# rvignav/diffusion-tts

Measured on AMD Instinct MI355X. Metric: candidate U-Net steps/sec, EDM ImageNet-64 eps-greedy N=64, higher is better.
Workload: dtype f16x3; 1 GPU; EDM ImageNet-64 (ADM 295.9M) eps-greedy search iteration, imagenet scorer, sigma step 5/18; candidates_total=64, candidates_per_gpu=64, scorer=imagenet, scorer_dtype=f16x3, denoiser_dtype=f16x3, graph_replay=True, parity_grade=True, parallelism=candidates sharded x1, 1 all-gather of rewards per step

## Files before the change

### diffusion_tts_amd/build.py

```python
import os
import re
import subprocess
import sys
from concurrent.futures import ThreadPoolExecutor

HERE = os.path.dirname(os.path.abspath(__file__))
CSRC = os.path.join(HERE, 'csrc')
LIB = os.path.join(HERE, 'libdts_hip.so')
SOURCES = ['conv_igemm.hip', 'conv_small.hip', 'groupnorm.hip', 'attention.hip', 'elementwise.hip', 'resample.hip', 'transformer.hip', 'group_rows.hip', 'vit.hip', 'jpeg.hip']
HIPCC = os.environ.get('HIPCC', '/opt/rocm/bin/hipcc')
FLAGS = ['--offload-arch=gfx950', '-O3', '-std=c++17', '-fPIC', '-Wall', '-Wno-unused-function']
EXTRA = {'attention.hip': ['-mllvm', '-amdgpu-mfma-vgpr-form=1']}


def _newer(a, b):
    return (not os.path.exists(b)) or os.path.getmtime(a) > os.path.getmtime(b)


def build(force=False, verbose=False):
    hdrs = [os.path.join(CSRC, 'dts_common.h'), os.path.join(HERE, '..', 'include', 'dts.h')]
    objs, jobs = [], []
    for src in SOURCES:
        s = os.path.join(CSRC, src)
        o = os.path.join(CSRC, src.replace('.hip', '.o'))
        objs.append(o)
        if force or _newer(s, o) or any(_newer(h, o) for h in hdrs):
            jobs.append([HIPCC, *FLAGS, *EXTRA.get(src, []), '-c', s, '-o', o])

    def run(cmd):
        if verbose:
            print(' '.join(cmd), flush=True)
        r = subprocess.run(cmd, capture_output=True, text=True)
        if r.returncode != 0:
            raise RuntimeError(f'hipcc failed: {" ".join(cmd)}\n{r.stdout}\n{r.stderr}')
        return r.stderr

    if jobs and os.path.exists(LIB):
        os.remove(LIB)
    with ThreadPoolExecutor(max_workers=4) as ex:
        for warn in ex.map(run, jobs):
            if verbose and warn.strip():
                print(warn)
    if jobs or force or not os.path.exists(LIB):
        for o in M0_OBJECTS:
            check_m0(os.path.join(CSRC, o))
        run([HIPCC, '--offload-arch=gfx950', '-shared', '-fPIC', '-o', LIB, *objs])
    return LIB


OBJDUMP = os.environ.get('LLVM_OBJDUMP', '/opt/rocm/lib/llvm/bin/llvm-objdump')
READELF = os.environ.get('LLVM_READELF', os.path.join(os.path.dirname(OBJDUMP), 'llvm-readelf'))
M0_OBJECTS = ['conv_igemm.o', 'attention.o']


def _device_object(obj, tmp):
    import glob
    local = os.path.join(tmp, os.path.basename(obj))
    with open(obj, 'rb') as f, open(local, 'wb') as g:
        g.write(f.read())
    subprocess.run([OBJDUMP, '--offloading', local], capture_output=True, text=True, cwd=tmp)
    dev = glob.glob(local + '.*gfx950*')
    if not dev:
        raise RuntimeError('no gfx950 code object found in ' + obj)
    return dev[0]


def check_m0(obj):
    import tempfile
    if not os.path.exists(OBJDUMP):
        print(f'WARNING: {OBJDUMP} not found: the M0 safety check of {os.path.basename(obj)} was SKIPPED (set LLVM_OBJDUMP)', file=sys.stderr)
        return -1
    with tempfile.TemporaryDirectory() as tmp:
        dev = _device_object(obj, tmp)
        dis = subprocess.run([OBJDUMP, '-d', dev], capture_output=True, text=True).stdout
        notes = subprocess.run([READELF, '--notes', dev], capture_output=True, text=True).stdout if os.path.exists(READELF) else ''
    name = os.path.basename(obj)
    ours = re.compile(r'^s_mov_b32 m0, (s\d+|vcc_lo|vcc_hi)$')
    uses, bad, dma_kernels, cur = 0, [], set(), None
    for ln in dis.splitlines():
        m = re.match(r'^[0-9a-f]+ <([^>]+)>:', ln)
        if m:
            cur = m.group(1)
            continue
        code = ln.split('//')[0].strip()
        if 'm0' in code:
            uses += 1
            dma_kernels.add(cur)
            if not ours.match(code):
                bad.append(code)
    if bad or not uses:
        raise RuntimeError(f'{name} code object: {len(bad)} instruction(s) other than our `s_mov_b32 m0, sN` use M0 '
                           f'(first: {bad[:3]}); the M0-clobber shortcut of the LDS-DMA helpers is no longer safe')
    if notes:
        spilled = []
        for blk in re.split(r'\n\s+- \.agpr_count', notes)[1:]:
            g = lambda k: re.search(r'\.%s:\s+(\S+)' % k, blk).group(1)
            if g('name') in dma_kernels and (int(g('private_segment_fixed_size')) != 0 or int(g('vgpr_spill_count')) != 0):
                spilled.append((g('name'), int(g('private_segment_fixed_size')), int(g('vgpr_spill_count'))))
        if spilled:
            raise RuntimeError(f'{name}: LDS-DMA kernels with scratch / VGPR spills (their hand-counted vmcnt waits would no longer hold): {spilled[:3]}')
    else:
        print(f'WARNING: {READELF} not found: the no-scratch check of the LDS-DMA kernels in {name} was SKIPPED', file=sys.stderr)
    return uses


if __name__ == '__main__':
    print(build(force='--force' in sys.argv, verbose=True))
```

### diffusion_tts_amd/csrc/attention.hip

```cpp
#include "dts_common.h"
#include <mutex>
#include <unordered_map>

namespace {

template <typename T> struct AttMma;
template <> struct AttMma<bf16_t> {
  static __device__ __forceinline__ f32x4_t run(const uint4& a, const uint4& b, f32x4_t c) {
    return __builtin_amdgcn_mfma_f32_16x16x32_bf16(__builtin_bit_cast(bf16x8_t, a), __builtin_bit_cast(bf16x8_t, b), c, 0, 0, 0);
  }
  static __device__ __forceinline__ uint32_t pack2(float lo, float hi) { return pack2_bf16(lo, hi); }
  static constexpr uint32_t ONES2 = 0x3F803F80u;
};
template <> struct AttMma<f16_t> {
  static __device__ __forceinline__ f32x4_t run(const uint4& a, const uint4& b, f32x4_t c) {
    return __builtin_amdgcn_mfma_f32_16x16x32_f16(__builtin_bit_cast(f16x8_t, a), __builtin_bit_cast(f16x8_t, b), c, 0, 0, 0);
  }
  static __device__ __forceinline__ uint32_t pack2(float lo, float hi) { return pack2_f16(lo, hi); }
  static constexpr uint32_t ONES2 = 0x3C003C00u;
};

__device__ __forceinline__ float vmax3(float a, float b, float c) {
  float r;
  asm("v_max3_f32 %0, %1, %2, %3" : "=v"(r) : "v"(a), "v"(b), "v"(c));
  return r;
}
__device__ __forceinline__ float vmax2(float a, float b) {
  float r;
  asm("v_max_f32 %0, %1, %2" : "=v"(r) : "v"(a), "v"(b));
  return r;
}

__device__ uint4 g_att_zero[64];

__device__ __forceinline__ void att_glds16(const char* g, uint32_t lds_off) {
  asm volatile("s_mov_b32 m0, %1\n\ts_nop 0\n\tglobal_load_lds_dwordx4 %0, off" : : "v"(g), "s"(lds_off) : "memory", "m0");
}

struct AttP {
  const char* qkv; char* out;
  int n, t, heads, d;
  float scale_log2e;
  int qblocks;
  int xcd_remap;
  int out_split3;
};

__device__ __forceinline__ void att_block(const AttP& p, int& nh, int& qb) {
  int bid = blockIdx.x;
  if (p.xcd_remap) {
    const int nblk = gridDim.x, q = nblk >> 3, r = nblk & 7, xcd = bid & 7, j = bid >> 3;
    bid = (xcd < r ? xcd * (q + 1) : r * (q + 1) + (xcd - r) * q) + j;
  }
  nh = bid / p.qblocks;
  qb = bid - nh * p.qblocks;
}

template <typename T, int D, int QT, int DV = D, bool PREF = true, bool DB = false, bool DMA = false>
__global__ __launch_bounds__(256) void attention16_kernel(const AttP p) {
  static_assert(!DB || PREF, "double buffering rides on the register prefetch");
  static_assert(!DMA || (D == 512 && DV == 256 && QT == 1 && !PREF && !DB), "LDS-DMA staging: the head-dim-512 form only");
  constexpr int ES = 2, ROWB = D * ES + 32;
  constexpr int VROWB = DV * ES + 32;
  constexpr int CH = D / 8;
  constexpr int CHV = DV / 8;
  constexpr int KSTEPS = D / 32;
  constexpr int DT = DV / 16;
  constexpr int NSL = D / DV;
  constexpr bool WIDE = DMA;
  extern __shared__ __attribute__((aligned(16))) char smem[];
  constexpr int BUFB = 64 * ROWB + 64 * VROWB;
  char* sK = smem;
  char* sV = smem + 64 * ROWB;
  const int tid = threadIdx.x, lane = tid & 63, wid = tid >> 6;
  const int lq = lane & 15, lg = lane >> 4;
  int nh, qblk;
  att_block(p, nh, qblk);
  int vs = 0;
  if constexpr (NSL > 1) { vs = nh % NSL; nh /= NSL; }
  const int n = nh / p.heads, head = nh - n * p.heads;
  const int C = p.heads * D;
  const size_t rowstride = (size_t)3 * C * ES;
  const char* base = p.qkv + (size_t)n * p.t * rowstride + (size_t)head * D * ES;
  const int q0 = qblk * (64 * QT) + wid * (16 * QT);

  uint4 qf[QT][KSTEPS];
#pragma unroll
  for (int qt = 0; qt < QT; ++qt)
#pragma unroll
    for (int s = 0; s < KSTEPS; ++s) {
      const int qrow = q0 + qt * 16 + lq;
      qf[qt][s] = make_uint4(0, 0, 0, 0);
      if (qrow < p.t) qf[qt][s] = *reinterpret_cast<const uint4*>(base + (size_t)qrow * rowstride + (lg + 4 * s) * 16);
    }
  const float sc2 = p.scale_log2e;
  f32x4_t o[QT][DT];
  f32x4_t ol[QT];
  const uint4 ones = make_uint4(AttMma<T>::ONES2, AttMma<T>::ONES2, AttMma<T>::ONES2, AttMma<T>::ONES2);
  float m_run[QT];
#pragma unroll
  for (int qt = 0; qt < QT; ++qt) {
    m_run[qt] = -INFINITY; ol[qt] = f32x4_t{0.f, 0.f, 0.f, 0.f};
#pragma unroll
    for (int i = 0; i < DT; ++i) o[qt][i] = f32x4_t{0.f, 0.f, 0.f, 0.f};
  }

  const int ntiles = (p.t + 63) / 64;
  constexpr int NCH = (64 * CH) / 256;
  constexpr int NCHV = (64 * CHV) / 256;
  constexpr int NPF = PREF ? NCH : 1, NPFV = PREF ? NCHV : 1;
  uint4 pk[NPF], pv[NPFV];
  const char* const vbase = base + (size_t)2 * C * ES + (size_t)vs * DV * ES;
#define ATT_LOAD_TILE(key0_)                                                                     \
  _Pragma("unroll") for (int u = 0; u < NCH; ++u) {                                               \
    const int idx = tid + 256 * u, r = idx / CH, c = idx - r * CH;                                \
    pk[u] = make_uint4(0, 0, 0, 0);                                                               \
    if ((key0_) + r < p.t) pk[u] = *reinterpret_cast<const uint4*>(base + (size_t)((key0_) + r) * rowstride + c * 16 + (size_t)C * ES); \
  }                                                                                               \
  _Pragma("unroll") for (int u = 0; u < NCHV; ++u) {                                              \
    const int idx = tid + 256 * u, r = idx / CHV, c = idx - r * CHV;                              \
    pv[u] = make_uint4(0, 0, 0, 0);                                                               \
    if ((key0_) + r < p.t) pv[u] = *reinterpret_cast<const uint4*>(vbase + (size_t)((key0_) + r) * rowstride + c * 16); \
  }
#define ATT_STAGE_TILE(boff_)                                                                     \
  _Pragma("unroll") for (int u = 0; u < NCH; ++u) {                                               \
    const int idx = tid + 256 * u, r = idx / CH, c = idx - r * CH;                                \
    *reinterpret_cast<uint4*>(sK + (boff_) + r * ROWB + c * 16) = pk[u];                          \
  }                                                                                               \
  _Pragma("unroll") for (int u = 0; u < NCHV; ++u) {                                              \
    const int idx = tid + 256 * u, r = idx / CHV, c = idx - r * CHV;                              \
    *reinterpret_cast<uint4*>(sV + (boff_) + r * VROWB + c * 16) = pv[u];                         \
  }
  const uint32_t lds_k = (uint32_t)(uintptr_t)(__attribute__((address_space(3))) char*)sK;
  const uint32_t lds_v = (uint32_t)(uintptr_t)(__attribute__((address_space(3))) char*)sV;
  const char* const zsrc = reinterpret_cast<const char*>(g_att_zero) + lane * 16;
#define ATT_DMA_K(key0_)                                                                         \
  _Pragma("unroll") for (int i = 0; i < 16; ++i) {                                                \
    const int r = wid * 16 + i;                                                                   \
    const char* src = ((key0_) + r < p.t) ? base + (size_t)((key0_) + r) * rowstride + (size_t)C * ES + lane * 16 : zsrc; \
    att_glds16(src, __builtin_amdgcn_readfirstlane(lds_k + r * ROWB));                            \
  }
#define ATT_DMA_V(key0_)                                                                         \
  if (lane < 32) {                                                                                \
    _Pragma("unroll") for (int i = 0; i < 16; ++i) {                                              \
      const int r = wid * 16 + i;                                                                 \
      const char* src = ((key0_) + r < p.t) ? vbase + (size_t)((key0_) + r) * rowstride + lane * 16 : zsrc; \
      att_glds16(src, __builtin_amdgcn_readfirstlane(lds_v + r * VROWB));                         \
    }                                                                                             \
  }
  if constexpr (DMA) { ATT_DMA_K(0); ATT_DMA_V(0); }
  if constexpr (PREF) { ATT_LOAD_TILE(0); }
  if constexpr (DB) {
    ATT_STAGE_TILE(0);
    if (ntiles > 1) { ATT_LOAD_TILE(64); }
  }
  for (int kt = 0; kt < ntiles; ++kt) {
    const int key0 = kt * 64;
    const int boff = DB ? (kt & 1) * BUFB : 0;
    if constexpr (DMA) asm volatile("s_waitcnt vmcnt(16)" ::: "memory");
    __syncthreads();
    if constexpr (DMA) {
    } else if constexpr (DB) {
      if (kt + 1 < ntiles) {
        ATT_STAGE_TILE(BUFB - boff);
        if (kt + 2 < ntiles) { ATT_LOAD_TILE(key0 + 128); }
      }
    } else if constexpr (PREF) {
      ATT_STAGE_TILE(0);
    } else {
#pragma unroll
      for (int u0 = 0; u0 < NCH; u0 += 4) {
        uint4 tk[4];
#pragma unroll
        for (int u = 0; u < 4; ++u) {
          const int idx = tid + 256 * (u0 + u), r = idx / CH, c = idx - r * CH;
          tk[u] = make_uint4(0, 0, 0, 0);
          if (key0 + r < p.t) tk[u] = *reinterpret_cast<const uint4*>(base + (size_t)(key0 + r) * rowstride + c * 16 + (size_t)C * ES);
        }
#pragma unroll
        for (int u = 0; u < 4; ++u) {
          const int idx = tid + 256 * (u0 + u), r = idx / CH, c = idx - r * CH;
          *reinterpret_cast<uint4*>(sK + r * ROWB + c * 16) = tk[u];
        }
      }
#pragma unroll
      for (int u0 = 0; u0 < NCHV; u0 += 4) {
        uint4 tv[4];
#pragma unroll
        for (int u = 0; u < 4; ++u) {
// ... 3 lines not shown
        }
#pragma unroll
        for (int u = 0; u < 4; ++u) {
          const int idx = tid + 256 * (u0 + u), r = idx / CHV, c = idx - r * CHV;
          *reinterpret_cast<uint4*>(sV + r * VROWB + c * 16) = tv[u];
        }
      }
    }
    if constexpr (!DB && !DMA) {
      __syncthreads();
      if constexpr (PREF) { if (kt + 1 < ntiles) { ATT_LOAD_TILE(key0 + 64); } }
    }

    f32x4_t sacc[QT][4];
    if constexpr (WIDE) {
#pragma unroll
      for (int j = 0; j < 4; ++j)
#pragma unroll
        for (int qt = 0; qt < QT; ++qt) sacc[qt][j] = f32x4_t{0.f, 0.f, 0.f, 0.f};
#pragma unroll
      for (int s = 0; s < KSTEPS; ++s) {
        uint4 ka[4];
#pragma unroll
        for (int j = 0; j < 4; ++j) ka[j] = *reinterpret_cast<const uint4*>(sK + boff + (j * 16 + lq) * ROWB + (lg + 4 * s) * 16);
#pragma unroll
        for (int j = 0; j < 4; ++j)
#pragma unroll
          for (int qt = 0; qt < QT; ++qt) sacc[qt][j] = AttMma<T>::run(ka[j], qf[qt][s], sacc[qt][j]);
      }
    } else {
#pragma unroll
    for (int j = 0; j < 4; ++j) {
#pragma unroll
      for (int qt = 0; qt < QT; ++qt) sacc[qt][j] = f32x4_t{0.f, 0.f, 0.f, 0.f};
#pragma unroll
      for (int s = 0; s < KSTEPS; ++s) {
        const uint4 ka = *reinterpret_cast<const uint4*>(sK + boff + (j * 16 + lq) * ROWB + (lg + 4 * s) * 16);
#pragma unroll
        for (int qt = 0; qt < QT; ++qt) sacc[qt][j] = AttMma<T>::run(ka, qf[qt][s], sacc[qt][j]);
      }
    }
    }
    if constexpr (DMA) {
      __syncthreads();
      if (kt + 1 < ntiles) { ATT_DMA_K(key0 + 64); }
    }
    uint4 pb[QT][2];
#pragma unroll
    for (int qt = 0; qt < QT; ++qt) {
      if (key0 + 64 > p.t) {
#pragma unroll
        for (int j = 0; j < 4; ++j)
#pragma unroll
          for (int r = 0; r < 4; ++r)
            if (key0 + j * 16 + lg * 4 + r >= p.t) sacc[qt][j][r] = -INFINITY;
      }
      float tmax = vmax3(sacc[qt][0][0], sacc[qt][0][1], sacc[qt][0][2]);
      tmax = vmax3(tmax, sacc[qt][0][3], sacc[qt][1][0]);
      tmax = vmax3(tmax, sacc[qt][1][1], sacc[qt][1][2]);
      tmax = vmax3(tmax, sacc[qt][1][3], sacc[qt][2][0]);
      tmax = vmax3(tmax, sacc[qt][2][1], sacc[qt][2][2]);
      tmax = vmax3(tmax, sacc[qt][2][3], sacc[qt][3][0]);
      tmax = vmax3(tmax, sacc[qt][3][1], sacc[qt][3][2]);
      tmax = vmax2(tmax, sacc[qt][3][3]);
      {
        const float t16 = __shfl_xor(tmax, 16, 64), t32 = __shfl_xor(tmax, 32, 64), t48 = __shfl_xor(tmax, 48, 64);
        tmax = vmax2(vmax3(tmax, t16, t32), t48);
      }
      const float m_new = vmax2(m_run[qt], tmax);
      const float alpha = __builtin_amdgcn_exp2f((m_run[qt] - m_new) * sc2);
      const float mb = m_new * sc2;
#pragma unroll
      for (int j = 0; j < 4; ++j)
#pragma unroll
        for (int r = 0; r < 4; ++r) sacc[qt][j][r] = __builtin_amdgcn_exp2f(fmaf(sacc[qt][j][r], sc2, -mb));
      m_run[qt] = m_new;
      if (!__all(alpha == 1.0f)) {
#pragma unroll
        for (int i = 0; i < DT; ++i) o[qt][i] *= alpha;
        ol[qt][0] *= alpha;
      }
#pragma unroll
      for (int kk = 0; kk < 2; ++kk) {
        pb[qt][kk].x = AttMma<T>::pack2(sacc[qt][2 * kk][0], sacc[qt][2 * kk][1]);
        pb[qt][kk].y = AttMma<T>::pack2(sacc[qt][2 * kk][2], sacc[qt][2 * kk][3]);
        pb[qt][kk].z = AttMma<T>::pack2(sacc[qt][2 * kk + 1][0], sacc[qt][2 * kk + 1][1]);
        pb[qt][kk].w = AttMma<T>::pack2(sacc[qt][2 * kk + 1][2], sacc[qt][2 * kk + 1][3]);
      }
    }

    if constexpr (DMA) {
      if (kt + 1 < ntiles) asm volatile("s_waitcnt vmcnt(16)" ::: "memory");
      else asm volatile("s_waitcnt vmcnt(0)" ::: "memory");
      __syncthreads();
    }
#pragma unroll
    for (int kk = 0; kk < 2; ++kk) {
      const int rq = (lane & 15) >> 2, rp = lane & 3;
      const char* va = sV + boff + (32 * kk + 4 * lg + rq) * VROWB + rp * 8;
#pragma unroll
      for (int qt = 0; qt < QT; ++qt) ol[qt] = AttMma<T>::run(ones, pb[qt][kk], ol[qt]);
      const char* vb = va + 16 * VROWB;
      if constexpr (WIDE) {
#pragma unroll
        for (int dt0 = 0; dt0 < DT; dt0 += 4) {
          uint4 av[4];
#pragma unroll
          for (int u = 0; u < 4; ++u) {
            const s16x4_t lo = __builtin_amdgcn_ds_read_tr16_b64_v4i16((__attribute__((address_space(3))) s16x4_t*)(va + (dt0 + u) * 32));
            const s16x4_t hi = __builtin_amdgcn_ds_read_tr16_b64_v4i16((__attribute__((address_space(3))) s16x4_t*)(vb + (dt0 + u) * 32));
            const uint2 lo2 = __builtin_bit_cast(uint2, lo), hi2 = __builtin_bit_cast(uint2, hi);
            av[u] = make_uint4(lo2.x, lo2.y, hi2.x, hi2.y);
          }
#pragma unroll
          for (int u = 0; u < 4; ++u)
#pragma unroll
            for (int qt = 0; qt < QT; ++qt) o[qt][dt0 + u] = AttMma<T>::run(av[u], pb[qt][kk], o[qt][dt0 + u]);
        }
      } else {
#pragma unroll
      for (int dt = 0; dt < DT; ++dt) {
        const s16x4_t lo = __builtin_amdgcn_ds_read_tr16_b64_v4i16((__attribute__((address_space(3))) s16x4_t*)(va + dt * 32));
        const s16x4_t hi = __builtin_amdgcn_ds_read_tr16_b64_v4i16((__attribute__((address_space(3))) s16x4_t*)(vb + dt * 32));
        const uint2 lo2 = __builtin_bit_cast(uint2, lo), hi2 = __builtin_bit_cast(uint2, hi);
        const uint4 av = make_uint4(lo2.x, lo2.y, hi2.x, hi2.y);
#pragma unroll
        for (int qt = 0; qt < QT; ++qt) o[qt][dt] = AttMma<T>::run(av, pb[qt][kk], o[qt][dt]);
      }
      }
    }
    if constexpr (DMA) {
      __syncthreads();
      if (kt + 1 < ntiles) { ATT_DMA_V(key0 + 64); }
    }
  }
#pragma unroll
  for (int qt = 0; qt < QT; ++qt) {
    const int qrow = q0 + qt * 16 + lq;
    if (qrow < p.t) {
      const float inv = 1.f / ol[qt][0];
      T* orow = reinterpret_cast<T*>(p.out) + ((size_t)n * p.t + qrow) * C + head * D + vs * DV;
#pragma unroll
      for (int dt = 0; dt < DT; ++dt)
#pragma unroll
        for (int r = 0; r < 4; ++r) st1<T>(orow + dt * 16 + lg * 4 + r, o[qt][dt][r] * inv);
    }
  }
}
#undef ATT_LOAD_TILE
#undef ATT_STAGE_TILE
#undef ATT_DMA_K
#undef ATT_DMA_V

template <int QT, int VAR = 7>
__global__ __launch_bounds__(256) void attention_x3_kernel(const AttP p) {
  using T = f16_t;
  constexpr bool KPRE = (VAR & 1) != 0, SM2 = (VAR & 2) != 0;
  constexpr int D = 64, ES = 2, ROWB = 2 * D * ES + 32, CH = 2 * D / 8, KSTEPS = D / 32, DT = D / 16, NCH = (64 * CH) / 256;
  extern __shared__ __attribute__((aligned(16))) char smem[];
  char* sK = smem;
  char* sV = smem + 64 * ROWB;
  const int tid = threadIdx.x, lane = tid & 63, wid = tid >> 6;
  const int lq = lane & 15, lg = lane >> 4;
  int nh, qblk;
  att_block(p, nh, qblk);
  const int n = nh / p.heads, head = nh - n * p.heads;
  const int C = p.heads * D;
  const size_t rowstride = (size_t)6 * C * ES;
  const size_t LO = (size_t)3 * C * ES;
  const char* base = p.qkv + (size_t)n * p.t * rowstride + (size_t)head * D * ES;
  const int q0 = qblk * (64 * QT) + wid * (16 * QT);
  uint4 qh[QT][KSTEPS], ql[QT][KSTEPS];
#pragma unroll
  for (int qt = 0; qt < QT; ++qt)
#pragma unroll
    for (int s = 0; s < KSTEPS; ++s) {
      const int qrow = q0 + qt * 16 + lq;
      qh[qt][s] = ql[qt][s] = make_uint4(0, 0, 0, 0);
      if (qrow < p.t) {
        qh[qt][s] = *reinterpret_cast<const uint4*>(base + (size_t)qrow * rowstride + (lg + 4 * s) * 16);
        ql[qt][s] = *reinterpret_cast<const uint4*>(base + (size_t)qrow * rowstride + LO + (lg + 4 * s) * 16);
      }
    }
  const float sc2 = p.scale_log2e * (1.0f / 4096.0f);
  f32x4_t o[QT][DT], ol[QT];
  const uint4 ones = make_uint4(AttMma<T>::ONES2, AttMma<T>::ONES2, AttMma<T>::ONES2, AttMma<T>::ONES2);
  float m_run[QT];
#pragma unroll
  for (int qt = 0; qt < QT; ++qt) {
    m_run[qt] = -INFINITY; ol[qt] = f32x4_t{0.f, 0.f, 0.f, 0.f};
#pragma unroll
    for (int i = 0; i < DT; ++i) o[qt][i] = f32x4_t{0.f, 0.f, 0.f, 0.f};
  }
  const int ntiles = (p.t + 63) / 64;
  uint4 pk[NCH], pv[NCH];
  static_assert(CH == 16 && NCH == 4, "tile staging layout");
  typedef unsigned int att_u32x4 __attribute__((ext_vector_type(4)));
  const __amdgpu_buffer_rsrc_t rs_kv = __builtin_amdgcn_make_buffer_rsrc((void*)const_cast<char*>(base), 0, 0x7fff0000, 0x00020000);
  uint32_t koff[NCH];
  {
    const int r = tid >> 4, c = tid & 15;
#pragma unroll
    for (int u = 0; u < NCH; ++u)
      koff[u] = (uint32_t)((size_t)(r + 16 * u) * rowstride + (c < 8 ? 0 : LO) + (size_t)(c & 7) * 16 + (size_t)C * ES);
  }
  const uint32_t v_plane = (uint32_t)((size_t)C * ES);
#define X3_LD(voff_, soff_) __builtin_bit_cast(uint4, (att_u32x4)__builtin_amdgcn_raw_buffer_load_b128(rs_kv, (int)(voff_), (int)(soff_), 0))
#define X3_LOAD_TILE(key0_)                                                                      \
  {                                                                                               \
    const uint32_t so_ = (uint32_t)((size_t)(key0_) * rowstride);                                 \
    if ((key0_) + 64 <= p.t) {                                                                    \
      _Pragma("unroll") for (int u = 0; u < NCH; ++u) { pk[u] = X3_LD(koff[u], so_); pv[u] = X3_LD(koff[u], so_ + v_plane); }      \
    } else {                                                                                      \
      _Pragma("unroll") for (int u = 0; u < NCH; ++u) {                                           \
        const uint32_t vo_ = ((key0_) + (tid >> 4) + 16 * u < p.t) ? koff[u] : 0x80000000u;       \
        pk[u] = X3_LD(vo_, so_); pv[u] = X3_LD(vo_, so_ + v_plane);                               \
      }                                                                                           \
    }                                                                                             \
  }
  const uint32_t st_off = (uint32_t)((tid >> 4) * ROWB + (tid & 15) * 16);
#define X3_STAGE_TILE()                                                                           \
  _Pragma("unroll") for (int u = 0; u < NCH; ++u) {                                               \
    *reinterpret_cast<uint4*>(sK + st_off + u * (16 * ROWB)) = pk[u];                             \
    *reinterpret_cast<uint4*>(sV + st_off + u * (16 * ROWB)) = pv[u];                             \
  }
  X3_LOAD_TILE(0);
  for (int kt = 0; kt < ntiles; ++kt) {
    const int key0 = kt * 64;
    __syncthreads();
    X3_STAGE_TILE();
    __syncthreads();
    if (kt + 1 < ntiles) { X3_LOAD_TILE(key0 + 64); }
    f32x4_t sacc[QT][4];
    uint4 kf[2][KSTEPS][2];
#pragma unroll
    for (int s = 0; s < KSTEPS; ++s) {
      kf[0][s][0] = *reinterpret_cast<const uint4*>(sK + lq * ROWB + (lg + 4 * s) * 16);
      kf[0][s][1] = *reinterpret_cast<const uint4*>(sK + lq * ROWB + D * ES + (lg + 4 * s) * 16);
    }
#pragma unroll
    for (int j = 0; j < 4; ++j) {
#pragma unroll
      for (int qt = 0; qt < QT; ++qt) sacc[qt][j] = f32x4_t{0.f, 0.f, 0.f, 0.f};
      if (KPRE && j < 3) {
#pragma unroll
        for (int s = 0; s < KSTEPS; ++s) {
          kf[(j + 1) & 1][s][0] = *reinterpret_cast<const uint4*>(sK + ((j + 1) * 16 + lq) * ROWB + (lg + 4 * s) * 16);
          kf[(j + 1) & 1][s][1] = *reinterpret_cast<const uint4*>(sK + ((j + 1) * 16 + lq) * ROWB + D * ES + (lg + 4 * s) * 16);
        }
      }
      if constexpr (KPRE) __builtin_amdgcn_sched_barrier(0);
#pragma unroll
      for (int s = 0; s < KSTEPS; ++s) {
        uint4 kh = kf[j & 1][s][0], kl = kf[j & 1][s][1];
        if (!KPRE && j > 0) {
          kh = *reinterpret_cast<const uint4*>(sK + (j * 16 + lq) * ROWB + (lg + 4 * s) * 16);
          kl = *reinterpret_cast<const uint4*>(sK + (j * 16 + lq) * ROWB + D * ES + (lg + 4 * s) * 16);
        }
#pragma unroll
        for (int qt = 0; qt < QT; ++qt) {
          sacc[qt][j] = AttMma<T>::run(kh, qh[qt][s], sacc[qt][j]);
          sacc[qt][j] = AttMma<T>::run(kh, ql[qt][s], sacc[qt][j]);
          sacc[qt][j] = AttMma<T>::run(kl, qh[qt][s], sacc[qt][j]);
        }
      }
    }
#define X3_VFRAG(kk_, dt_, avh_, avl_)                                                                                                    \
  {                                                                                                                                       \
    const char* va_ = sV + (32 * (kk_) + 4 * lg + ((lane & 15) >> 2)) * ROWB + (lane & 3) * 8 + (dt_) * 32;                                \
    const uint2 h0_ = __builtin_bit_cast(uint2, __builtin_amdgcn_ds_read_tr16_b64_v4i16((__attribute__((address_space(3))) s16x4_t*)(va_)));               \
    const uint2 h1_ = __builtin_bit_cast(uint2, __builtin_amdgcn_ds_read_tr16_b64_v4i16((__attribute__((address_space(3))) s16x4_t*)(va_ + 16 * ROWB)));   \
    const uint2 l0_ = __builtin_bit_cast(uint2, __builtin_amdgcn_ds_read_tr16_b64_v4i16((__attribute__((address_space(3))) s16x4_t*)(va_ + D * ES)));      \
    const uint2 l1_ = __builtin_bit_cast(uint2, __builtin_amdgcn_ds_read_tr16_b64_v4i16((__attribute__((address_space(3))) s16x4_t*)(va_ + 16 * ROWB + D * ES))); \
    avh_ = make_uint4(h0_.x, h0_.y, h1_.x, h1_.y); avl_ = make_uint4(l0_.x, l0_.y, l1_.x, l1_.y);                                          \
  }
    constexpr int VPRE = (VAR & 4) ? 2 : 0;
    uint4 vpre[VPRE > 0 ? VPRE : 1][2];
#pragma unroll
    for (int dt = 0; dt < VPRE; ++dt) X3_VFRAG(0, dt, vpre[dt][0], vpre[dt][1]);
    uint4 pbh[QT][2], pbl[QT][2];
    float tmx[QT], t16[QT], t32[QT], t48[QT];
#pragma unroll
    for (int qt = 0; qt < QT; ++qt) {
      if (key0 + 64 > p.t) {
#pragma unroll
        for (int j = 0; j < 4; ++j)
#pragma unroll
          for (int r = 0; r < 4; ++r)
            if (key0 + j * 16 + lg * 4 + r >= p.t) sacc[qt][j][r] = -INFINITY;
      }
      float tmax = vmax3(sacc[qt][0][0], sacc[qt][0][1], sacc[qt][0][2]);
      tmax = vmax3(tmax, sacc[qt][0][3], sacc[qt][1][0]);
      tmax = vmax3(tmax, sacc[qt][1][1], sacc[qt][1][2]);
      tmax = vmax3(tmax, sacc[qt][1][3], sacc[qt][2][0]);
      tmax = vmax3(tmax, sacc[qt][2][1], sacc[qt][2][2]);
      tmax = vmax3(tmax, sacc[qt][2][3], sacc[qt][3][0]);
      tmax = vmax3(tmax, sacc[qt][3][1], sacc[qt][3][2]);
      tmx[qt] = vmax2(tmax, sacc[qt][3][3]);
    }
    if constexpr (SM2) {
#pragma unroll
      for (int qt = 0; qt < QT; ++qt) {
        t16[qt] = __shfl_xor(tmx[qt], 16, 64); t32[qt] = __shfl_xor(tmx[qt], 32, 64); t48[qt] = __shfl_xor(tmx[qt], 48, 64);
      }
    }
#pragma unroll
    for (int qt = 0; qt < QT; ++qt) {
      float tmax;
      if constexpr (SM2) tmax = vmax2(vmax3(tmx[qt], t16[qt], t32[qt]), t48[qt]);
      else { tmax = vmax2(tmx[qt], __shfl_xor(tmx[qt], 16, 64)); tmax = vmax2(tmax, __shfl_xor(tmax, 32, 64)); }
      const float m_new = vmax2(m_run[qt], tmax);
      const float alpha = __builtin_amdgcn_exp2f((m_run[qt] - m_new) * sc2);
      const float mb = m_new * sc2 - 14.0f;
      m_run[qt] = m_new;
      if (!__all(alpha == 1.0f)) {
#pragma unroll
        for (int i = 0; i < DT; ++i) o[qt][i] *= alpha;
        ol[qt][0] *= alpha;
      }
      uint32_t hw_[4][2], lw_[4][2];
#pragma unroll
      for (int j = 0; j < 4; ++j)
#pragma unroll
        for (int r = 0; r < 4; r += 2) {
          const float e0 = __builtin_amdgcn_exp2f(fmaf(sacc[qt][j][r], sc2, -mb));
          const float e1 = __builtin_amdgcn_exp2f(fmaf(sacc[qt][j][r + 1], sc2, -mb));
          const dts_f32x2_t ev = {e0, e1};
          const dts_f16x2_t hv = __builtin_convertvector(ev, dts_f16x2_t);
          const float l0 = __builtin_fmaf((float)hv[0], -1.0f, e0), l1 = __builtin_fmaf((float)hv[1], -1.0f, e1);
          hw_[j][r >> 1] = __builtin_bit_cast(uint32_t, hv);
          lw_[j][r >> 1] = pack2_f16(l0, l1);
        }
#pragma unroll
      for (int kk = 0; kk < 2; ++kk) {
        pbh[qt][kk] = make_uint4(hw_[2 * kk][0], hw_[2 * kk][1], hw_[2 * kk + 1][0], hw_[2 * kk + 1][1]);
        pbl[qt][kk] = make_uint4(lw_[2 * kk][0], lw_[2 * kk][1], lw_[2 * kk + 1][0], lw_[2 * kk + 1][1]);
      }
    }
#pragma unroll
    for (int kk = 0; kk < 2; ++kk) {
#pragma unroll
      for (int qt = 0; qt < QT; ++qt) {
        ol[qt] = AttMma<T>::run(ones, pbh[qt][kk], ol[qt]);
        ol[qt] = AttMma<T>::run(ones, pbl[qt][kk], ol[qt]);
      }
#pragma unroll
      for (int dt = 0; dt < DT; ++dt) {
        uint4 avh, avl;
        if (kk == 0 && dt < VPRE) { avh = vpre[dt][0]; avl = vpre[dt][1]; }
        else X3_VFRAG(kk, dt, avh, avl);
#pragma unroll
        for (int qt = 0; qt < QT; ++qt) {
          o[qt][dt] = AttMma<T>::run(avh, pbh[qt][kk], o[qt][dt]);
          o[qt][dt] = AttMma<T>::run(avh, pbl[qt][kk], o[qt][dt]);
          o[qt][dt] = AttMma<T>::run(avl, pbh[qt][kk], o[qt][dt]);
        }
      }
    }
  }
#undef X3_VFRAG
#undef X3_LOAD_TILE
#undef X3_LD
#undef X3_STAGE_TILE
#pragma unroll
  for (int qt = 0; qt < QT; ++qt) {
    const int qrow = q0 + qt * 16 + lq;
    if (qrow < p.t) {
      const float inv = (1.0f / 64.0f) / ol[qt][0];
      if (p.out_split3) {
        f16_t* orow3 = reinterpret_cast<f16_t*>(p.out) + ((size_t)n * p.t + qrow) * 2 * C;
#pragma unroll
        for (int dt = 0; dt < DT; ++dt) {
          float hi[4], lo[4];
#pragma unroll
          for (int r = 0; r < 4; ++r) {
            float x = o[qt][dt][r] * inv;
            asm volatile("" : "+v"(x));
            x3_split(x, hi[r], lo[r]);
          }
          f16_t* d_ = orow3 + x3_off(head * D + dt * 16 + lg * 4);
          *reinterpret_cast<uint2*>(d_) = make_uint2(pack2_f16(hi[0], hi[1]), pack2_f16(hi[2], hi[3]));
          *reinterpret_cast<uint2*>(d_ + 32) = make_uint2(pack2_f16(lo[0], lo[1]), pack2_f16(lo[2], lo[3]));
        }
      } else {
        float* orow = reinterpret_cast<float*>(p.out) + ((size_t)n * p.t + qrow) * C + head * D;
#pragma unroll
        for (int dt = 0; dt < DT; ++dt)
          *reinterpret_cast<float4*>(orow + dt * 16 + lg * 4) = make_float4(o[qt][dt][0] * inv, o[qt][dt][1] * inv, o[qt][dt][2] * inv, o[qt][dt][3] * inv);
      }
    }
  }
}


template <int D>
__global__ __launch_bounds__(256) void attention32_kernel(const AttP p) {
  constexpr int ES = 4, ROWB = D * ES + 32;
  constexpr int CH = D / 4;
  constexpr int KCH = D / 16;
  constexpr int DT = D / 16;
  extern __shared__ __attribute__((aligned(16))) char smem[];
  char* sK = smem;
  char* sV = smem + 64 * ROWB;
  const int tid = threadIdx.x, lane = tid & 63, wid = tid >> 6;
  const int lq = lane & 15, lg = lane >> 4;
  int nh, qblk;
  att_block(p, nh, qblk);
  const int n = nh / p.heads, head = nh - n * p.heads;
  const int C = p.heads * D;
  const size_t rowstride = (size_t)3 * C * ES;
  const char* base = p.qkv + (size_t)n * p.t * rowstride + (size_t)head * D * ES;
  const int q0 = qblk * 64 + wid * 16;
  const int qrow = q0 + lq;

  f32x4_t o[DT];
#pragma unroll
  for (int i = 0; i < DT; ++i) o[i] = f32x4_t{0.f, 0.f, 0.f, 0.f};
  float m_run = -INFINITY, l_run = 0.f;
  const int ntiles = (p.t + 63) / 64;
  for (int kt = 0; kt < ntiles; ++kt) {
    const int key0 = kt * 64;
    __syncthreads();
    for (int idx = tid; idx < 64 * CH; idx += 256) {
      const int r = idx / CH, c = idx - r * CH;
      uint4 kv = make_uint4(0, 0, 0, 0), vv = make_uint4(0, 0, 0, 0);
      if (key0 + r < p.t) {
        const char* g = base + (size_t)(key0 + r) * rowstride + c * 16;
        kv = *reinterpret_cast<const uint4*>(g + (size_t)C * ES);
        vv = *reinterpret_cast<const uint4*>(g + (size_t)2 * C * ES);
      }
      *reinterpret_cast<uint4*>(sK + r * ROWB + c * 16) = kv;
      *reinterpret_cast<uint4*>(sV + r * ROWB + c * 16) = vv;
    }
    __syncthreads();
    f32x4_t sacc[4];
#pragma unroll
    for (int j = 0; j < 4; ++j) sacc[j] = f32x4_t{0.f, 0.f, 0.f, 0.f};
#pragma unroll
    for (int s = 0; s < KCH; ++s) {
      float4 qv = make_float4(0.f, 0.f, 0.f, 0.f);
      if (qrow < p.t) qv = *reinterpret_cast<const float4*>(base + (size_t)qrow * rowstride + (lg + 4 * s) * 16);
#pragma unroll
      for (int j = 0; j < 4; ++j) {
        const float4 ka = *reinterpret_cast<const float4*>(sK + (j * 16 + lq) * ROWB + (lg + 4 * s) * 16);
        sacc[j] = __builtin_amdgcn_mfma_f32_16x16x4f32(ka.x, qv.x, sacc[j], 0, 0, 0);
        sacc[j] = __builtin_amdgcn_mfma_f32_16x16x4f32(ka.y, qv.y, sacc[j], 0, 0, 0);
        sacc[j] = __builtin_amdgcn_mfma_f32_16x16x4f32(ka.z, qv.z, sacc[j], 0, 0, 0);
        sacc[j] = __builtin_amdgcn_mfma_f32_16x16x4f32(ka.w, qv.w, sacc[j], 0, 0, 0);
      }
    }
    float tmax = -INFINITY;
#pragma unroll
    for (int j = 0; j < 4; ++j)
#pragma unroll
      for (int r = 0; r < 4; ++r) {
        float v = sacc[j][r] * p.scale_log2e;
        if (key0 + j * 16 + lg * 4 + r >= p.t) v = -INFINITY;
        sacc[j][r] = v;
        tmax = fmaxf(tmax, v);
      }
    tmax = fmaxf(tmax, __shfl_xor(tmax, 16, 64));
    tmax = fmaxf(tmax, __shfl_xor(tmax, 32, 64));
    const float m_new = fmaxf(m_run, tmax);
    const float alpha = exp2f(m_run - m_new);
    float psum = 0.f;
#pragma unroll
    for (int j = 0; j < 4; ++j)
#pragma unroll
      for (int r = 0; r < 4; ++r) {
        const float e = exp2f(sacc[j][r] - m_new);
        sacc[j][r] = e;
        psum += e;
      }
    psum += __shfl_xor(psum, 16, 64);
    psum += __shfl_xor(psum, 32, 64);
    l_run = l_run * alpha + psum;
    m_run = m_new;
#pragma unroll
    for (int i = 0; i < DT; ++i) o[i] *= alpha;
#pragma unroll
    for (int j = 0; j < 4; ++j)
#pragma unroll
      for (int r = 0; r < 4; ++r) {
        const char* vrow = sV + (j * 16 + 4 * lg + r) * ROWB + lq * 4;
#pragma unroll
        for (int dt = 0; dt < DT; ++dt) {
          const float va = *reinterpret_cast<const float*>(vrow + dt * 64);
          o[dt] = __builtin_amdgcn_mfma_f32_16x16x4f32(va, sacc[j][r], o[dt], 0, 0, 0);
        }
      }
  }
  if (qrow < p.t) {
    const float inv = 1.f / l_run;
    float* orow = reinterpret_cast<float*>(p.out) + ((size_t)n * p.t + qrow) * C + head * D;
#pragma unroll
    for (int dt = 0; dt < DT; ++dt) {
      const float4 v = make_float4(o[dt][0] * inv, o[dt][1] * inv, o[dt][2] * inv, o[dt][3] * inv);
      *reinterpret_cast<float4*>(orow + dt * 16 + lg * 4) = v;
    }
  }
}

struct AttMaskP {
  const char* qkv; char* out;
  const int32_t* key_len;
  int n, t, heads;
  float scale_log2e;
  int qblocks, xcd_remap, causal;
};

template <typename T>
__global__ __launch_bounds__(256) void attention_masked_kernel(const AttMaskP p) {
  constexpr int D = 64, ES = 2, ROWB = D * ES + 32, CH = D / 8, KSTEPS = D / 32, DT = D / 16, NCH = (64 * CH) / 256;
// ... 58 lines not shown
    if (kt + 1 < ntiles) { ATTM_LOAD_TILE(key0 + 64); }

    f32x4_t sacc[4];
#pragma unroll
    for (int j = 0; j < 4; ++j) {
      sacc[j] = f32x4_t{0.f, 0.f, 0.f, 0.f};
#pragma unroll
      for (int s = 0; s < KSTEPS; ++s) {
        const uint4 ka = *reinterpret_cast<const uint4*>(sK + (j * 16 + lq) * ROWB + (lg + 4 * s) * 16);
        sacc[j] = AttMma<T>::run(ka, qf[s], sacc[j]);
      }
    }
    if (key0 + 64 > kend || (p.causal && key0 + 63 > q0)) {
#pragma unroll
      for (int j = 0; j < 4; ++j)
#pragma unroll
        for (int r = 0; r < 4; ++r)
          if (key0 + j * 16 + lg * 4 + r >= lim) sacc[j][r] = -INFINITY;
    }
    float tmax = vmax3(sacc[0][0], sacc[0][1], sacc[0][2]);
    tmax = vmax3(tmax, sacc[0][3], sacc[1][0]);
    tmax = vmax3(tmax, sacc[1][1], sacc[1][2]);
    tmax = vmax3(tmax, sacc[1][3], sacc[2][0]);
    tmax = vmax3(tmax, sacc[2][1], sacc[2][2]);
    tmax = vmax3(tmax, sacc[2][3], sacc[3][0]);
    tmax = vmax3(tmax, sacc[3][1], sacc[3][2]);
    tmax = vmax2(tmax, sacc[3][3]);
    {
      const float t16 = __shfl_xor(tmax, 16, 64), t32 = __shfl_xor(tmax, 32, 64), t48 = __shfl_xor(tmax, 48, 64);
      tmax = vmax2(vmax3(tmax, t16, t32), t48);
    }
    const float m_new = vmax2(m_run, tmax);
    const float alpha = __builtin_amdgcn_exp2f((m_run - m_new) * sc2);
    const float mb = m_new * sc2;
#pragma unroll
    for (int j = 0; j < 4; ++j)
#pragma unroll
      for (int r = 0; r < 4; ++r) sacc[j][r] = __builtin_amdgcn_exp2f(fmaf(sacc[j][r], sc2, -mb));
    m_run = m_new;
    if (!__all(alpha == 1.0f)) {
#pragma unroll
      for (int i = 0; i < DT; ++i) o[i] *= alpha;
      ol[0] *= alpha;
    }
    uint4 pb[2];
#pragma unroll
    for (int kk = 0; kk < 2; ++kk) {
      pb[kk].x = AttMma<T>::pack2(sacc[2 * kk][0], sacc[2 * kk][1]);
      pb[kk].y = AttMma<T>::pack2(sacc[2 * kk][2], sacc[2 * kk][3]);
      pb[kk].z = AttMma<T>::pack2(sacc[2 * kk + 1][0], sacc[2 * kk + 1][1]);
      pb[kk].w = AttMma<T>::pack2(sacc[2 * kk + 1][2], sacc[2 * kk + 1][3]);
    }
#pragma unroll
    for (int kk = 0; kk < 2; ++kk) {
      const int rq = (lane & 15) >> 2, rp = lane & 3;
      const char* va = sV + (32 * kk + 4 * lg + rq) * ROWB + rp * 8;
      const char* vb = va + 16 * ROWB;
      ol = AttMma<T>::run(ones, pb[kk], ol);
#pragma unroll
      for (int dt = 0; dt < DT; ++dt) {
        const s16x4_t lo = __builtin_amdgcn_ds_read_tr16_b64_v4i16((__attribute__((address_space(3))) s16x4_t*)(va + dt * 32));
        const s16x4_t hi = __builtin_amdgcn_ds_read_tr16_b64_v4i16((__attribute__((address_space(3))) s16x4_t*)(vb + dt * 32));
        const uint2 lo2 = __builtin_bit_cast(uint2, lo), hi2 = __builtin_bit_cast(uint2, hi);
        o[dt] = AttMma<T>::run(make_uint4(lo2.x, lo2.y, hi2.x, hi2.y), pb[kk], o[dt]);
      }
    }
  }
#undef ATTM_LOAD_TILE
  if (qrow < p.t) {
    const float inv = 1.f / ol[0];
    T* orow = reinterpret_cast<T*>(p.out) + ((size_t)n * p.t + qrow) * C + head * D;
#pragma unroll
    for (int dt = 0; dt < DT; ++dt)
#pragma unroll
      for (int r = 0; r < 4; ++r) st1<T>(orow + dt * 16 + lg * 4 + r, o[dt][r] * inv);
  }
}

template <typename T>
int att_masked(AttMaskP p, hipStream_t st) {
  p.qblocks = (p.t + 63) / 64;
  p.xcd_remap = dts_knob_get(DTS_KNOB_ATT_XCD) != 0;
  const long long nblk = (long long)p.qblocks * p.n * p.heads;
  DTS_CHECK_ARG(nblk < (1ll << 31), "dts_attention_masked: grid too large");
  hipLaunchKernelGGL(attention_masked_kernel<T>, dim3((unsigned)nblk), dim3(256), 0, st, p);
  DTS_CHECK_LAUNCH("dts_attention_masked");
  return DTS_OK;
}

template <typename K>
int launch_att(K kernel, const AttP& p0, size_t lds, hipStream_t st, int qblock = 64, int slices = 1) {
  {
    static std::mutex mu;
    static std::unordered_map<uintptr_t, size_t> done;
    int dev = 0;
    if (hipGetDevice(&dev) != hipSuccess) dev = 0;
    std::lock_guard<std::mutex> lk(mu);
    size_t& have = done[reinterpret_cast<uintptr_t>(reinterpret_cast<const void*>(kernel)) ^ ((uintptr_t)(dev + 1) << 56)];
    if (lds > have) {
      (void)hipFuncSetAttribute(reinterpret_cast<const void*>(kernel), hipFuncAttributeMaxDynamicSharedMemorySize, (int)lds);
      have = lds;
    }
  }
  AttP p = p0;
  p.qblocks = (p.t + qblock - 1) / qblock;
  p.xcd_remap = dts_knob_get(DTS_KNOB_ATT_XCD) != 0;
  const long long nblk = (long long)p.qblocks * p.n * p.heads * slices;
  DTS_CHECK_ARG(nblk < (1ll << 31), "dts_attention: grid too large");
  hipLaunchKernelGGL(kernel, dim3((unsigned)nblk), dim3(256), lds, st, p);
  DTS_CHECK_LAUNCH("dts_attention");
  return DTS_OK;
}

template <typename T>
int att16(const AttP& p, hipStream_t st) {
  const int g_att_qt = dts_knob_get(DTS_KNOB_ATT_QT) > 0 ? dts_knob_get(DTS_KNOB_ATT_QT) : 0;
  const size_t lds = (size_t)2 * 64 * (p.d * 2 + 32);
  const bool db = dts_knob_get(DTS_KNOB_ATT_DB) == 1 && p.t > 64;
  switch (p.d) {
    case 64:
      if (g_att_qt == 2 || (g_att_qt == 0 && p.t >= 256 && (long long)((p.t + 127) / 128) * p.n * p.heads >= 512))
        return db ? launch_att(attention16_kernel<T, 64, 2, 64, true, true>, p, 2 * lds, st, 128)
                  : launch_att(attention16_kernel<T, 64, 2>, p, lds, st, 128);
      return db ? launch_att(attention16_kernel<T, 64, 1, 64, true, true>, p, 2 * lds, st) : launch_att(attention16_kernel<T, 64, 1>, p, lds, st);
    case 128:
      return db ? launch_att(attention16_kernel<T, 128, 1, 128, true, true>, p, 2 * lds, st) : launch_att(attention16_kernel<T, 128, 1>, p, lds, st);
    case 256: return launch_att(attention16_kernel<T, 256, 1>, p, lds, st);
    case 512:
      if (dts_knob_get(DTS_KNOB_ATT_DB) == 2)
        return launch_att(attention16_kernel<T, 512, 1, 256, false>, p, (size_t)64 * (512 * 2 + 32) + (size_t)64 * (256 * 2 + 32), st, 64, 2);
      return launch_att(attention16_kernel<T, 512, 1, 256, false, false, true>, p, (size_t)64 * (512 * 2 + 32) + (size_t)64 * (256 * 2 + 32), st, 64, 2);
  }
  return DTS_ERR_UNSUPPORTED;
}

int att32(const AttP& p, hipStream_t st) {
  const size_t lds = (size_t)2 * 64 * (p.d * 4 + 32);
  switch (p.d) {
    case 64: return launch_att(attention32_kernel<64>, p, lds, st);
    case 128: return launch_att(attention32_kernel<128>, p, lds, st);
    case 256: return launch_att(attention32_kernel<256>, p, lds, st);
  }
  return DTS_ERR_UNSUPPORTED;
}

}

extern "C" int dts_attention_x3(const void* qkv_split, void* out, int out_split3, int n, int t, int heads, int d, float scale, dts_stream s) {
  DTS_CHECK_ARG(qkv_split && out, "dts_attention_x3: null pointer");
  DTS_CHECK_ARG(n > 0 && t > 0 && heads > 0, "dts_attention_x3: bad shape");
  DTS_CHECK_ARG(d == 64, "dts_attention_x3: head dim %d unsupported (64; other sizes take dts_attention in DTS_F32)", d);
  DTS_CHECK_ARG((long long)t * 6 * heads * d * 2 < (1ll << 31), "dts_attention_x3: %d tokens x %d heads exceed the 2 GiB a sample's rows may span", t, heads);
  AttP p{(const char*)qkv_split, (char*)out, n, t, heads, d, scale * 1.4426950408889634f, 0, 1, out_split3 ? 1 : 0};
  const size_t lds = (size_t)2 * 64 * (2 * 64 * 2 + 32);
  const int qt = dts_knob_get(DTS_KNOB_ATT_QT);
  const bool two = qt == 2 || (qt != 1 && t >= 512 && (long long)((t + 127) / 128) * n * heads >= 512);
  const int var = (dts_knob_get(DTS_KNOB_ATT_DB) >= 16 && dts_knob_get(DTS_KNOB_ATT_DB) < 32) ? dts_knob_get(DTS_KNOB_ATT_DB) - 16 : 7;
#define X3_LAUNCH(V_) (two ? launch_att(attention_x3_kernel<2, V_>, p, lds, to_stream(s), 128) : launch_att(attention_x3_kernel<1, V_>, p, lds, to_stream(s)))
  if (var == 0) return X3_LAUNCH(0);
  return X3_LAUNCH(7);
#undef X3_LAUNCH
}

extern "C" int dts_attention_masked(const void* qkv, void* out, int dtype, int n, int t, int heads, int d, float scale, int causal,
                                    const int32_t* key_len, dts_stream s) {
  DTS_CHECK_ARG(qkv && out, "dts_attention_masked: null pointer");
  DTS_CHECK_ARG(n > 0 && t > 0 && heads > 0, "dts_attention_masked: bad shape");
  DTS_CHECK_ARG(dtype == DTS_F32 || dtype == DTS_BF16 || dtype == DTS_F16, "dts_attention_masked: bad dtype %d", dtype);
  DTS_CHECK_ARG(scale > 0.f && scale <= 3.402823466e38f, "dts_attention_masked: scale must be positive and finite");
  DTS_CHECK_ARG(((uintptr_t)qkv | (uintptr_t)out) % 16 == 0 && (uintptr_t)key_len % 4 == 0, "dts_attention_masked: pointers must be 16-byte aligned");
  if (dtype == DTS_F32) {
    dts_set_error("dts_attention_masked: dtype %d (DTS_F32) unsupported (DTS_BF16 / DTS_F16 only)", dtype);
    return DTS_ERR_UNSUPPORTED;
  }
  if (d != 64) {
    dts_set_error("dts_attention_masked: head dim %d unsupported (64, the head dim of every CLIP text width)", d);
    return DTS_ERR_UNSUPPORTED;
  }
  AttMaskP p{(const char*)qkv, (char*)out, key_len, n, t, heads, scale * 1.4426950408889634f, 0, 1, causal ? 1 : 0};
  return dtype == DTS_BF16 ? att_masked<bf16_t>(p, to_stream(s)) : att_masked<f16_t>(p, to_stream(s));
}

extern "C" int dts_attention(const void* qkv, void* out, int dtype, int n, int t, int heads, int d, float scale, dts_stream s) {
  DTS_CHECK_ARG(qkv && out, "dts_attention: null pointer");
  DTS_CHECK_ARG(n > 0 && t > 0 && heads > 0, "dts_attention: bad shape");
  DTS_CHECK_ARG(d == 64 || d == 128 || d == 256 || (d == 512 && dtype != DTS_F32),
                "dts_attention: head dim %d unsupported (64/128/256; 512 in the 16-bit types)", d);
  AttP p{(const char*)qkv, (char*)out, n, t, heads, d, scale * 1.4426950408889634f, 0, 1, 0};
  hipStream_t st = to_stream(s);
  switch (dtype) {
    case DTS_F32: return att32(p, st);
    case DTS_BF16: return att16<bf16_t>(p, st);
    case DTS_F16: return att16<f16_t>(p, st);
  }
  dts_set_error("dts_attention: bad dtype %d", dtype);
  return DTS_ERR_ARG;
}
```

Before: 1428 candidate U-Net steps/sec.

## Stage x3 attention K/V tiles via LDS-DMA with swizzled layout

```diff
diff --git a/diffusion_tts_amd/build.py b/diffusion_tts_amd/build.py
--- a/diffusion_tts_amd/build.py
+++ b/diffusion_tts_amd/build.py
@@ -44,6 +44,7 @@
     if jobs or force or not os.path.exists(LIB):
         for o in M0_OBJECTS:
             check_m0(os.path.join(CSRC, o))
+        check_att_x3_regs(os.path.join(CSRC, 'attention.o'))
         run([HIPCC, '--offload-arch=gfx950', '-shared', '-fPIC', '-o', LIB, *objs])
     return LIB
 
@@ -104,5 +105,30 @@
     return uses
 
 
+X3_DMA_VGPRS = {2: 168, 1: 128}
+
+
+def check_att_x3_regs(obj):
+    import tempfile
+    if not (os.path.exists(OBJDUMP) and os.path.exists(READELF)):
+        print(f'WARNING: {OBJDUMP} / {READELF} not found: the register budget check of attention_x3_kernel was SKIPPED', file=sys.stderr)
+        return {}
+    with tempfile.TemporaryDirectory() as tmp:
+        notes = subprocess.run([READELF, '--notes', _device_object(obj, tmp)], capture_output=True, text=True).stdout
+    seen, over = {}, []
+    for blk in re.split(r'\n\s+- \.agpr_count', notes)[1:]:
+        name = re.search(r'\.name:\s+(\S+)', blk).group(1)
+        m = re.search(r'attention_x3_kernelILi(\d+)ELi\d+ELb1E', name)
+        if not m:
+            continue
+        seen[name] = int(re.search(r'\.vgpr_count:\s+(\d+)', blk).group(1)) + int(re.match(r':\s+(\d+)', blk).group(1))
+        if seen[name] > X3_DMA_VGPRS[int(m.group(1))]:
+            over.append((name, seen[name], X3_DMA_VGPRS[int(m.group(1))]))
+    if over or not seen:
+        raise RuntimeError(f'attention.o: LDS-DMA forms of attention_x3_kernel over their register budget (kernel, registers, budget): {over}'
+                           if over else 'attention.o: no LDS-DMA form of attention_x3_kernel found in the code object')
+    return seen
+
+
 if __name__ == '__main__':
     print(build(force='--force' in sys.argv, verbose=True))
diff --git a/diffusion_tts_amd/csrc/attention.hip b/diffusion_tts_amd/csrc/attention.hip
--- a/diffusion_tts_amd/csrc/attention.hip
+++ b/diffusion_tts_amd/csrc/attention.hip
@@ -35,6 +35,10 @@
 
 __device__ __forceinline__ void att_glds16(const char* g, uint32_t lds_off) {
   asm volatile("s_mov_b32 m0, %1\n\ts_nop 0\n\tglobal_load_lds_dwordx4 %0, off" : : "v"(g), "s"(lds_off) : "memory", "m0");
+}
+
+__device__ __forceinline__ void att_glds16s(const char* sbase, uint32_t voff, uint32_t lds_off) {
+  asm volatile("s_mov_b32 m0, %2\n\ts_nop 0\n\tglobal_load_lds_dwordx4 %0, %1" : : "v"(voff), "s"(sbase), "s"(lds_off) : "memory", "m0");
 }
 
 struct AttP {
@@ -344,16 +348,21 @@
 #undef ATT_DMA_K
 #undef ATT_DMA_V
 
-template <int QT, int VAR = 7>
+constexpr int X3_WAIT_VM0_LGKM0 = 0x0070;
+template <int QT, int VAR = 7, bool DMA = false>
 __global__ __launch_bounds__(256) void attention_x3_kernel(const AttP p) {
   using T = f16_t;
   constexpr bool KPRE = (VAR & 1) != 0, SM2 = (VAR & 2) != 0;
-  constexpr int D = 64, ES = 2, ROWB = 2 * D * ES + 32, CH = 2 * D / 8, KSTEPS = D / 32, DT = D / 16, NCH = (64 * CH) / 256;
+  constexpr int D = 64, ES = 2, ROWB = DMA ? D * ES : 2 * D * ES + 32, CH = 2 * D / 8, KSTEPS = D / 32, DT = D / 16, NCH = (64 * CH) / 256;
+  constexpr int LOB = DMA ? 64 * D * ES : D * ES;
+  constexpr int TILEB = DMA ? 2 * 64 * D * ES : 64 * ROWB;
   extern __shared__ __attribute__((aligned(16))) char smem[];
   char* sK = smem;
-  char* sV = smem + 64 * ROWB;
+  char* sV = smem + TILEB;
   const int tid = threadIdx.x, lane = tid & 63, wid = tid >> 6;
   const int lq = lane & 15, lg = lane >> 4;
+  const uint32_t ksw = DMA ? (uint32_t)((lq >> 1) & 3) << 5 : 0u;
+  const uint32_t vsw = DMA ? (uint32_t)(((4 * lg + ((lane & 15) >> 2)) >> 1) & 3) << 5 : 0u;
   int nh, qblk;
   att_block(p, nh, qblk);
   const int n = nh / p.heads, head = nh - n * p.heads;
@@ -385,7 +394,7 @@
     for (int i = 0; i < DT; ++i) o[qt][i] = f32x4_t{0.f, 0.f, 0.f, 0.f};
   }
   const int ntiles = (p.t + 63) / 64;
-  uint4 pk[NCH], pv[NCH];
+  uint4 pk[DMA ? 1 : NCH], pv[DMA ? 1 : NCH];
   static_assert(CH == 16 && NCH == 4, "tile staging layout");
   typedef unsigned int att_u32x4 __attribute__((ext_vector_type(4)));
   const __amdgpu_buffer_rsrc_t rs_kv = __builtin_amdgcn_make_buffer_rsrc((void*)const_cast<char*>(base), 0, 0x7fff0000, 0x00020000);
@@ -416,19 +425,49 @@
     *reinterpret_cast<uint4*>(sK + st_off + u * (16 * ROWB)) = pk[u];                             \
     *reinterpret_cast<uint4*>(sV + st_off + u * (16 * ROWB)) = pv[u];                             \
   }
-  X3_LOAD_TILE(0);
+  const uint32_t lds_k = (uint32_t)(uintptr_t)(__attribute__((address_space(3))) char*)sK + (uint32_t)(wid & 1) * 1024u + (uint32_t)(wid >> 1) * LOB;
+  const uint32_t lds_v = lds_k + TILEB;
+  const int dma_row = 8 * (wid & 1) + (lane >> 3);
+  const uint32_t dma_c = (uint32_t)(lane & 7) ^ ((uint32_t)((dma_row >> 1) & 3) << 1);
+  const uint32_t dma_off = (uint32_t)((size_t)dma_row * rowstride + (size_t)(wid >> 1) * LO + (size_t)dma_c * 16 + (size_t)C * ES);
+  const char* const zsrc = reinterpret_cast<const char*>(g_att_zero) + lane * 16;
+#define X3_DMA_TILE(lds_, key0_, plane_)                                                          \
+  {                                                                                               \
+    const char* sb_ = base + (size_t)(key0_) * rowstride + (plane_);                              \
+    if ((key0_) + 64 <= p.t) {                                                                    \
+      _Pragma("unroll") for (int u = 0; u < 4; ++u)                                               \
+        att_glds16s(sb_ + (size_t)(16 * u) * rowstride, dma_off, __builtin_amdgcn_readfirstlane((lds_) + u * 2048));    \
+    } else {                                                                                      \
+      _Pragma("unroll") for (int u = 0; u < 4; ++u) {                                             \
+        const char* src_ = ((key0_) + 16 * u + dma_row < p.t) ? sb_ + (size_t)(16 * u) * rowstride + dma_off : zsrc;    \
+        att_glds16(src_, __builtin_amdgcn_readfirstlane((lds_) + u * 2048));                      \
+      }                                                                                           \
+    }                                                                                             \
+  }
+  if constexpr (DMA) {
+    X3_DMA_TILE(lds_k, 0, 0);
+  } else {
+    X3_LOAD_TILE(0);
+  }
   for (int kt = 0; kt < ntiles; ++kt) {
     const int key0 = kt * 64;
-    __syncthreads();
-    X3_STAGE_TILE();
-    __syncthreads();
-    if (kt + 1 < ntiles) { X3_LOAD_TILE(key0 + 64); }
+    if constexpr (DMA) {
+      __builtin_amdgcn_s_waitcnt(X3_WAIT_VM0_LGKM0);
+      __syncthreads();
+      X3_DMA_TILE(lds_v, key0, v_plane);
+    } else {
+      __syncthreads();
+      X3_STAGE_TILE();
+      __syncthreads();
+      if (kt + 1 < ntiles) { X3_LOAD_TILE(key0 + 64); }
+    }
     f32x4_t sacc[QT][4];
+#define X3_KADDR(j_, s_, lo_) (sK + ((j_) * 16 + lq) * ROWB + ((uint32_t)((lg + 4 * (s_)) * 16) ^ ksw) + (lo_) * LOB)
     uint4 kf[2][KSTEPS][2];
 #pragma unroll
     for (int s = 0; s < KSTEPS; ++s) {
-      kf[0][s][0] = *reinterpret_cast<const uint4*>(sK + lq * ROWB + (lg + 4 * s) * 16);
-      kf[0][s][1] = *reinterpret_cast<const uint4*>(sK + lq * ROWB + D * ES + (lg + 4 * s) * 16);
+      kf[0][s][0] = *reinterpret_cast<const uint4*>(X3_KADDR(0, s, 0));
+      kf[0][s][1] = *reinterpret_cast<const uint4*>(X3_KADDR(0, s, 1));
     }
 #pragma unroll
     for (int j = 0; j < 4; ++j) {
@@ -437,8 +476,8 @@
       if (KPRE && j < 3) {
 #pragma unroll
         for (int s = 0; s < KSTEPS; ++s) {
-          kf[(j + 1) & 1][s][0] = *reinterpret_cast<const uint4*>(sK + ((j + 1) * 16 + lq) * ROWB + (lg + 4 * s) * 16);
-          kf[(j + 1) & 1][s][1] = *reinterpret_cast<const uint4*>(sK + ((j + 1) * 16 + lq) * ROWB + D * ES + (lg + 4 * s) * 16);
+          kf[(j + 1) & 1][s][0] = *reinterpret_cast<const uint4*>(X3_KADDR(j + 1, s, 0));
+          kf[(j + 1) & 1][s][1] = *reinterpret_cast<const uint4*>(X3_KADDR(j + 1, s, 1));
         }
       }
       if constexpr (KPRE) __builtin_amdgcn_sched_barrier(0);
@@ -446,8 +485,8 @@
       for (int s = 0; s < KSTEPS; ++s) {
         uint4 kh = kf[j & 1][s][0], kl = kf[j & 1][s][1];
         if (!KPRE && j > 0) {
-          kh = *reinterpret_cast<const uint4*>(sK + (j * 16 + lq) * ROWB + (lg + 4 * s) * 16);
-          kl = *reinterpret_cast<const uint4*>(sK + (j * 16 + lq) * ROWB + D * ES + (lg + 4 * s) * 16);
+          kh = *reinterpret_cast<const uint4*>(X3_KADDR(j, s, 0));
+          kl = *reinterpret_cast<const uint4*>(X3_KADDR(j, s, 1));
         }
 #pragma unroll
         for (int qt = 0; qt < QT; ++qt) {
@@ -457,13 +496,20 @@
         }
       }
     }
+    if constexpr (DMA) {
+      __builtin_amdgcn_s_waitcnt(X3_WAIT_VM0_LGKM0);
+      __syncthreads();
+      if (kt + 1 < ntiles) { X3_DMA_TILE(lds_k, key0 + 64, 0); }
+    }
 #define X3_VFRAG(kk_, dt_, avh_, avl_)                                                                                                    \
   {                                                                                                                                       \
-    const char* va_ = sV + (32 * (kk_) + 4 * lg + ((lane & 15) >> 2)) * ROWB + (lane & 3) * 8 + (dt_) * 32;                                \
-    const uint2 h0_ = __builtin_bit_cast(uint2, __builtin_amdgcn_ds_read_tr16_b64_v4i16((__attribute__((address_space(3))) s16x4_t*)(va_)));               \
-    const uint2 h1_ = __builtin_bit_cast(uint2, __builtin_amdgcn_ds_read_tr16_b64_v4i16((__attribute__((address_space(3))) s16x4_t*)(va_ + 16 * ROWB)));   \
-    const uint2 l0_ = __builtin_bit_cast(uint2, __builtin_amdgcn_ds_read_tr16_b64_v4i16((__attribute__((address_space(3))) s16x4_t*)(va_ + D * ES)));      \
-    const uint2 l1_ = __builtin_bit_cast(uint2, __builtin_amdgcn_ds_read_tr16_b64_v4i16((__attribute__((address_space(3))) s16x4_t*)(va_ + 16 * ROWB + D * ES))); \
+    const char* vr_ = sV + (32 * (kk_) + 4 * lg + ((lane & 15) >> 2)) * ROWB;                                                         \
+    const char* vh_ = vr_ + ((uint32_t)((lane & 3) * 8 + (dt_) * 32) ^ vsw);                                                               \
+    const char* vl_ = vh_ + LOB;                                                                                                           \
+    const uint2 h0_ = __builtin_bit_cast(uint2, __builtin_amdgcn_ds_read_tr16_b64_v4i16((__attribute__((address_space(3))) s16x4_t*)(vh_)));               \
+    const uint2 h1_ = __builtin_bit_cast(uint2, __builtin_amdgcn_ds_read_tr16_b64_v4i16((__attribute__((address_space(3))) s16x4_t*)(vh_ + 16 * ROWB)));   \
+    const uint2 l0_ = __builtin_bit_cast(uint2, __builtin_amdgcn_ds_read_tr16_b64_v4i16((__attribute__((address_space(3))) s16x4_t*)(vl_)));               \
+    const uint2 l1_ = __builtin_bit_cast(uint2, __builtin_amdgcn_ds_read_tr16_b64_v4i16((__attribute__((address_space(3))) s16x4_t*)(vl_ + 16 * ROWB)));   \
     avh_ = make_uint4(h0_.x, h0_.y, h1_.x, h1_.y); avl_ = make_uint4(l0_.x, l0_.y, l1_.x, l1_.y);                                          \
   }
     constexpr int VPRE = (VAR & 4) ? 2 : 0;
@@ -551,6 +597,8 @@
     }
   }
 #undef X3_VFRAG
+#undef X3_KADDR
+#undef X3_DMA_TILE
 #undef X3_LOAD_TILE
 #undef X3_LD
 #undef X3_STAGE_TILE
@@ -915,13 +963,15 @@
   DTS_CHECK_ARG(d == 64, "dts_attention_x3: head dim %d unsupported (64; other sizes take dts_attention in DTS_F32)", d);
   DTS_CHECK_ARG((long long)t * 6 * heads * d * 2 < (1ll << 31), "dts_attention_x3: %d tokens x %d heads exceed the 2 GiB a sample's rows may span", t, heads);
   AttP p{(const char*)qkv_split, (char*)out, n, t, heads, d, scale * 1.4426950408889634f, 0, 1, out_split3 ? 1 : 0};
-  const size_t lds = (size_t)2 * 64 * (2 * 64 * 2 + 32);
   const int qt = dts_knob_get(DTS_KNOB_ATT_QT);
   const bool two = qt == 2 || (qt != 1 && t >= 512 && (long long)((t + 127) / 128) * n * heads >= 512);
-  const int var = (dts_knob_get(DTS_KNOB_ATT_DB) >= 16 && dts_knob_get(DTS_KNOB_ATT_DB) < 32) ? dts_knob_get(DTS_KNOB_ATT_DB) - 16 : 7;
-#define X3_LAUNCH(V_) (two ? launch_att(attention_x3_kernel<2, V_>, p, lds, to_stream(s), 128) : launch_att(attention_x3_kernel<1, V_>, p, lds, to_stream(s)))
-  if (var == 0) return X3_LAUNCH(0);
-  return X3_LAUNCH(7);
+  const int db = dts_knob_get(DTS_KNOB_ATT_DB);
+  const int var = (db >= 16 && db < 32) ? db - 16 : 7;
+  const bool dma = !(db >= 16 && db < 32);
+  const size_t lds = dma ? (size_t)2 * 64 * 256 : (size_t)2 * 64 * (2 * 64 * 2 + 32);
+#define X3_LAUNCH(V_, M_) (two ? launch_att(attention_x3_kernel<2, V_, M_>, p, lds, to_stream(s), 128) : launch_att(attention_x3_kernel<1, V_, M_>, p, lds, to_stream(s)))
+  if (var == 0) return X3_LAUNCH(0, false);
+  return dma ? X3_LAUNCH(7, true) : X3_LAUNCH(7, false);
 #undef X3_LAUNCH
 }
 
```

Result: no change. 1439 candidate U-Net steps/sec, median of 6 (+0.8%).
